# Somedaywilldo/BM-NAS

Hardware: AMD Instinct MI355X
Metric: search-steps/sec (fwd+bwd of fusion hypernet) on MM-IMDB synthetic (higher is better)
Workload: dtype f32; 1 GPU; mmimdb fusion search, batch 128 per GPU x 1 GPU(s), N6 C192 L16 steps2 node_steps1 node_multiplier1, train mode, dropout 0.1/0.1(attn); inputs=(b, C, L) features, global_batch=128, per_gpu_batch=128, parallelism=dp1, mode=graph, step=fwd+bwd, one hipGraph replay

## Files before the change

bm-nas_amd/csrc/common.hpp:

```cpp
#pragma once
#include <hip/hip_runtime.h>
#include <stdint.h>

#define BMNAS_MAX_PTRS 16
#define BMNAS_WAVE 64

typedef __attribute__((ext_vector_type(4))) float f32x4;

struct PtrsIn { const float* p[BMNAS_MAX_PTRS]; };
struct PtrsOut { float* p[BMNAS_MAX_PTRS]; };

struct DropCfg {
  uint32_t thr;
  float scale;
  uint64_t seed;
  uint64_t offset;
  const uint64_t* step;
};

#define BMNAS_CHECK_LAUNCH()                         \
  do {                                               \
    hipError_t e__ = hipGetLastError();              \
    if (e__ != hipSuccess) return (int)e__;          \
  } while (0)

__device__ __forceinline__ uint4 philox4x32_10(uint64_t ctr, uint64_t seed) {
  uint32_t k0 = (uint32_t)seed, k1 = (uint32_t)(seed >> 32);
  uint32_t c0 = (uint32_t)ctr, c1 = (uint32_t)(ctr >> 32), c2 = 0x2545F491u, c3 = 0x9E3779B1u;
#pragma unroll
  for (int r = 0; r < 10; ++r) {
    uint32_t hi0 = __umulhi(0xD2511F53u, c0), lo0 = 0xD2511F53u * c0;
    uint32_t hi1 = __umulhi(0xCD9E8D57u, c2), lo1 = 0xCD9E8D57u * c2;
    uint32_t n0 = hi1 ^ c1 ^ k0, n1 = lo1, n2 = hi0 ^ c3 ^ k1, n3 = lo0;
    c0 = n0; c1 = n1; c2 = n2; c3 = n3;
    k0 += 0x9E3779B9u; k1 += 0xBB67AE85u;
  }
  return make_uint4(c0, c1, c2, c3);
}

struct DropRt {
  uint32_t thr;
  float scale;
  uint64_t seed;
  uint64_t off;
};
__device__ __forceinline__ DropRt drop_begin(const DropCfg& d) {
  DropRt r{d.thr, d.scale, d.seed, d.offset};
  if (d.thr != 0u && d.step != nullptr) r.off += d.step[0];
  return r;
}
__device__ __forceinline__ float4 drop_mult4(const DropRt& d, uint64_t e) {
  if (d.thr == 0u) return make_float4(1.f, 1.f, 1.f, 1.f);
  uint4 r = philox4x32_10(d.off + (e >> 2), d.seed);
  return make_float4(r.x >= d.thr ? d.scale : 0.f, r.y >= d.thr ? d.scale : 0.f,
                     r.z >= d.thr ? d.scale : 0.f, r.w >= d.thr ? d.scale : 0.f);
}

__device__ __forceinline__ float4 drop_mult4(const DropCfg& d, uint64_t e) {
  if (d.thr == 0u) return make_float4(1.f, 1.f, 1.f, 1.f);
  const uint64_t base = (d.step != nullptr) ? d.step[0] : 0ull;
  uint4 r = philox4x32_10(base + d.offset + (e >> 2), d.seed);
  return make_float4(r.x >= d.thr ? d.scale : 0.f, r.y >= d.thr ? d.scale : 0.f,
                     r.z >= d.thr ? d.scale : 0.f, r.w >= d.thr ? d.scale : 0.f);
}

#ifndef BMNAS_BODY_PROBES
#define BMNAS_BODY_PROBES 0
#endif
#if BMNAS_BODY_PROBES
static __device__ unsigned long long* g_bmnas_stamps = nullptr;
static __device__ int g_bmnas_stamp_slots = 0;
#define BMNAS_DEFINE_STAMP_SETTER(name)                                                                   \
  extern "C" int name(void* buf, int slots) {                                                             \
    unsigned long long* p = reinterpret_cast<unsigned long long*>(buf);                                   \
    if (hipMemcpyToSymbol(HIP_SYMBOL(g_bmnas_stamps), &p, sizeof(p)) != hipSuccess) return -1;            \
    if (hipMemcpyToSymbol(HIP_SYMBOL(g_bmnas_stamp_slots), &slots, sizeof(slots)) != hipSuccess) return -1; \
    return 0;                                                                                             \
  }
__device__ __forceinline__ unsigned long long stamp_clock() {
  unsigned long long t;
  asm volatile("s_memtime %0\n\ts_waitcnt lgkmcnt(0)" : "=s"(t)::"memory");
  return t;
}
__device__ __forceinline__ unsigned long long stamp_wall() {
  unsigned long long t;
  asm volatile("s_memrealtime %0\n\ts_waitcnt lgkmcnt(0)" : "=s"(t)::"memory");
  return t;
}
#define STAMP(slot, wg, i)                                                                         \
  do {                                                                                             \
    __builtin_amdgcn_sched_barrier(0);                                                             \
    if (threadIdx.x == 0 && g_bmnas_stamps != nullptr && (wg) < g_bmnas_stamp_slots) {             \
      unsigned long long* p__ = g_bmnas_stamps + ((size_t)(slot) * g_bmnas_stamp_slots + (wg)) * 8; \
      p__[i] = stamp_clock();                                                                      \
      if ((i) == 0) p__[6] = stamp_wall();                                                         \
      p__[7] = stamp_wall();                                                                       \
    }                                                                                              \
    __builtin_amdgcn_sched_barrier(0);                                                             \
  } while (0)
#else
#define STAMP(slot, wg, i) do { } while (0)
#define BMNAS_DEFINE_STAMP_SETTER(name) \
  extern "C" int name(void* buf, int slots) { (void)buf; (void)slots; return -3;  }
#endif

template <int CTRL>
__device__ __forceinline__ float dpp_f(float v) {
  return __int_as_float(__builtin_amdgcn_update_dpp(__float_as_int(v), __float_as_int(v), CTRL, 0xf, 0xf, false));
}
__device__ __forceinline__ float lane_xor1(float v) { return dpp_f<0xB1>(v); }
__device__ __forceinline__ float lane_xor2(float v) { return dpp_f<0x4E>(v); }
__device__ __forceinline__ float xor16_sum(float v) {
  auto r = __builtin_amdgcn_permlane16_swap(__float_as_uint(v), __float_as_uint(v), false, false);
  return __uint_as_float(r[0]) + __uint_as_float(r[1]);
}
__device__ __forceinline__ float xor32_sum(float v) {
  auto r = __builtin_amdgcn_permlane32_swap(__float_as_uint(v), __float_as_uint(v), false, false);
  return __uint_as_float(r[0]) + __uint_as_float(r[1]);
}
__device__ __forceinline__ float xor16_max(float v) {
  auto r = __builtin_amdgcn_permlane16_swap(__float_as_uint(v), __float_as_uint(v), false, false);
  return fmaxf(__uint_as_float(r[0]), __uint_as_float(r[1]));
}
__device__ __forceinline__ float xor32_max(float v) {
  auto r = __builtin_amdgcn_permlane32_swap(__float_as_uint(v), __float_as_uint(v), false, false);
  return fmaxf(__uint_as_float(r[0]), __uint_as_float(r[1]));
}
__device__ __forceinline__ float row_stride4_sum(float v) {
  v += dpp_f<0x124>(v);
  v += dpp_f<0x128>(v);
  return v;
}
__device__ __forceinline__ float row16_sum(float v) {
// ... 35 lines not shown

template <int NW>
__device__ __forceinline__ float block_sum_fresh(float v, float* red) {
  v = wave_sum(v);
  if ((threadIdx.x & 63) == 0) red[threadIdx.x >> 6] = v;
  __syncthreads();
  float t = red[0];
#pragma unroll
  for (int i = 1; i < NW; ++i) t += red[i];
  return t;
}

template <int NW, int N>
__device__ __forceinline__ void block_sum_lead_fresh(float (&v)[N], float* red) {
#pragma unroll
  for (int i = 0; i < N; ++i) v[i] = wave_sum(v[i]);
  const int w = threadIdx.x >> 6;
  if ((threadIdx.x & 63) == 0) {
#pragma unroll
    for (int i = 0; i < N; ++i) red[i * NW + w] = v[i];
  }
  __syncthreads();
  float t = red[0];
#pragma unroll
  for (int k = 1; k < NW; ++k) t += red[k];
  v[0] = t;
  if (threadIdx.x == 0) {
#pragma unroll
    for (int i = 1; i < N; ++i) {
      float u = red[i * NW];
#pragma unroll
      for (int k = 1; k < NW; ++k) u += red[i * NW + k];
      v[i] = u;
    }
  }
}

template <int NW, int N>
__device__ __forceinline__ void block_sum_n(float (&v)[N], float* red) {
#pragma unroll
  for (int i = 0; i < N; ++i) v[i] = wave_sum(v[i]);
  const int w = threadIdx.x >> 6;
  __syncthreads();
  if ((threadIdx.x & 63) == 0) {
#pragma unroll
    for (int i = 0; i < N; ++i) red[w * N + i] = v[i];
  }
  __syncthreads();
#pragma unroll
  for (int i = 0; i < N; ++i) {
    float t = red[i];
#pragma unroll
    for (int k = 1; k < NW; ++k) t += red[k * N + i];
    v[i] = t;
  }
}

template <int NW, int N>
__device__ __forceinline__ void block_sum_lead(float (&v)[N], float* red) {
  __syncthreads();
  block_sum_lead_fresh<NW, N>(v, red);
}

template <typename T>
__device__ __forceinline__ T* sgpr_ptr(T* p) {
  asm volatile("" : "+s"(p));
  return p;
}
template <typename T, int N>
__device__ __forceinline__ T* pick_ptr(T* const (&arr)[N], int q) {
  T* p = sgpr_ptr(arr[0]);
#pragma unroll
  for (int qq = 1; qq < N; ++qq) {
    T* c = sgpr_ptr(arr[qq]);
    p = (q == qq) ? c : p;
  }
  return p;
}

__device__ __forceinline__ float4 ld4(const float* p) { return *reinterpret_cast<const float4*>(p); }
__device__ __forceinline__ void st4(float* p, float4 v) { *reinterpret_cast<float4*>(p) = v; }
__device__ __forceinline__ void pin4(float4& v) { asm volatile("" : "+v"(v.x), "+v"(v.y), "+v"(v.z), "+v"(v.w)); }
__device__ __forceinline__ void pin1(float& v) { asm volatile("" : "+v"(v)); }

__device__ __forceinline__ void st4_wt(float* p, float4 v) {
#if defined(BMNAS_NO_WT)
  *reinterpret_cast<float4*>(p) = v;
#else
  const f32x4 d = {v.x, v.y, v.z, v.w};
  asm volatile("global_store_dwordx4 %0, %1, off sc1\n\ts_nop 1" : : "v"(p), "v"(d) : "memory");
#endif
}

#ifndef BMNAS_WT_MASK
#define BMNAS_WT_MASK 0x29
#endif
template <int G>
__device__ __forceinline__ void st4_wtg(float* p, float4 v) {
  if constexpr ((BMNAS_WT_MASK >> G) & 1) st4_wt(p, v);
  else *reinterpret_cast<float4*>(p) = v;
}

#ifndef BMNAS_WT0_MASK
#define BMNAS_WT0_MASK 0x7FF
#endif
template <int K>
__device__ __forceinline__ void st4_w0(float* p, float4 v) {
  if constexpr ((BMNAS_WT0_MASK >> K) & 1) st4_wt(p, v);
  else *reinterpret_cast<float4*>(p) = v;
}

__device__ __forceinline__ void st16_wt(void* p, uint4 v) {
#if defined(BMNAS_NO_WT) || !((BMNAS_WT_MASK >> 5) & 1)
  *reinterpret_cast<uint4*>(p) = v;
#else
  typedef __attribute__((ext_vector_type(4))) unsigned u32x4_;
  const u32x4_ d = {v.x, v.y, v.z, v.w};
  asm volatile("global_store_dwordx4 %0, %1, off sc1\n\ts_nop 1" : : "v"(p), "v"(d) : "memory");
#endif
}

__device__ __forceinline__ float4 f4_add(float4 a, float4 b) {
  return make_float4(a.x + b.x, a.y + b.y, a.z + b.z, a.w + b.w);
}
__device__ __forceinline__ float4 f4_mul(float4 a, float4 b) {
  return make_float4(a.x * b.x, a.y * b.y, a.z * b.z, a.w * b.w);
}
__device__ __forceinline__ float4 f4_scale(float4 a, float s) {
  return make_float4(a.x * s, a.y * s, a.z * s, a.w * s);
}
__device__ __forceinline__ float f4_dot(float4 a, float4 b) {
  return a.x * b.x + a.y * b.y + a.z * b.z + a.w * b.w;
}
__device__ __forceinline__ float f4_hsum(float4 a) { return (a.x + a.y) + (a.z + a.w); }

static inline int ilog2_exact(int v) {
  int l = 0;
  while ((1 << l) < v) ++l;
  return ((1 << l) == v) ? l : -1;
}
```

bm-nas_amd/csrc/head.hip:

```cpp
#include "common.hpp"
#include "../../include/bmnas_hip.h"
#include "lazy_ln.hpp"
#include "ln_sample.hpp"
#include <algorithm>
#include <cstdlib>

namespace {

constexpr int kHeadSrc = 4;
constexpr int kMaxO = 128;

struct HeadSrc {
  const float* p[kHeadSrc];
  const float* sums[kHeadSrc];
};

struct HeadLazy {
  const float* rec;
  const float* prm;
  const float* nw[kHeadSrc];
  const float* nb[kHeadSrc];
  float* nstats[kHeadSrc];
  float* lnpart[kHeadSrc];
  int lq, P;
};

__device__ __forceinline__ void sample_stats(const HeadSrc& src, int n_src, int s, int D, float* mean, float* rstd) {
  float S = 0.f, Q = 0.f;
  float2 sv[kHeadSrc];
#pragma unroll
  for (int q = 0; q < kHeadSrc; ++q)
    sv[q] = reinterpret_cast<const float2*>(pick_ptr(src.sums, q < n_src ? q : 0))[s];
#pragma unroll
  for (int q = 0; q < kHeadSrc; ++q) {
    S += q < n_src ? sv[q].x : 0.f;
    Q += q < n_src ? sv[q].y : 0.f;
  }
  const float inv = 1.f / (float)D;
  const float m = S * inv;
  const float var = fmaxf(Q * inv - m * m, 0.f);
  *mean = m;
  *rstd = 1.f / sqrtf(var + kLnEps);
}

struct HeadFwdArgs {
  HeadSrc src;
  const float* ln_w;
  const float* ln_b;
  const float* W;
  const float* bias;
  float* hb;
  float* hb_part;
  long long hb_stride;
  float* stats;
  int b, O, D, CL, n_src, KS;
};

template <int J, int TJ, bool LZ>
__global__ __launch_bounds__(256) void head_fwd_k(HeadFwdArgs a, HeadLazy z) {
  __shared__ float red[4][3][16][16 * TJ + 1];
  const int wave = threadIdx.x >> 6, lane = threadIdx.x & 63;
  const int lo = lane & 15, h = lane >> 4;
  const int ks = blockIdx.x, st = blockIdx.y;
  STAMP(4, blockIdx.y * gridDim.x + blockIdx.x, 0);
  const int s = st * 16 + lo;
  const int sc = s < a.b ? s : a.b - 1;
  const int nkb = a.D / 16;
  int oc[TJ];
#pragma unroll
  for (int t = 0; t < TJ; ++t) {
    const int o = 16 * t + lo;
    oc[t] = o < a.O ? o : a.O - 1;
  }
  float4 xv[J], lw[J], lb[J], wv[J][TJ], nwv[LZ ? J : 1], nbv[LZ ? J : 1];
  bool valid[J], lzq[J];
#pragma unroll
  for (int j = 0; j < J; ++j) {
    const int kb = (j * a.KS + ks) * 4 + wave;
    valid[j] = kb < nkb;
    const int kbc = valid[j] ? kb : nkb - 1;
    const int k = kbc * 16 + 4 * h;
    const int q = (kbc * 16) / a.CL;
    xv[j] = ld4(pick_ptr(a.src.p, q) + (int64_t)sc * a.CL + (k - q * a.CL));
    lw[j] = ld4(a.ln_w + k);
    lb[j] = ld4(a.ln_b + k);
    lzq[j] = LZ && q == z.lq;
    if (LZ) {
      nwv[j] = ld4(lzq[j] ? z.nw[0] + (k - q * a.CL) : a.ln_w + k);
      nbv[j] = ld4(lzq[j] ? z.nb[0] + (k - q * a.CL) : a.ln_b + k);
    }
#pragma unroll
    for (int t = 0; t < TJ; ++t) wv[j][t] = ld4(a.W + (int64_t)oc[t] * a.D + k);
  }
  __builtin_amdgcn_sched_barrier(0);
  float mean, rstd, nmean = 0.f, nrstd = 1.f;
  if (LZ) {
    float2 sv[kHeadSrc];
#pragma unroll
    for (int q = 0; q < kHeadSrc; ++q) {
      const bool use = q < a.n_src && q != z.lq;
      const int qq = use ? q : (z.lq == 0 ? (a.n_src > 1 ? 1 : 0) : 0);
      const float* sp = pick_ptr(a.src.sums, qq);
      sv[q] = reinterpret_cast<const float2*>(sp != nullptr ? sp : z.rec)[sc];
    }
    const LazyStats ls = lazy_combine(z.rec, z.prm, z.P, sc);
    float S = ls.osum, Q = ls.osq;
#pragma unroll
    for (int q = 0; q < kHeadSrc; ++q) {
      const bool use = q < a.n_src && q != z.lq;
      S += use ? sv[q].x : 0.f;
      Q += use ? sv[q].y : 0.f;
    }
    const float inv = 1.f / (float)a.D;
    mean = S * inv;
    rstd = 1.f / sqrtf(fmaxf(Q * inv - mean * mean, 0.f) + kLnEps);
    nmean = ls.mean;
    nrstd = ls.rstd;
  } else {
    sample_stats(a.src, a.n_src, sc, a.D, &mean, &rstd);
  }
  if (ks == 0 && wave == 0 && h == 0 && s < a.b) {
    a.stats[2 * s] = mean;
    a.stats[2 * s + 1] = rstd;
    if (LZ) {
      z.nstats[0][2 * s] = nmean;
      z.nstats[0][2 * s + 1] = nrstd;
    }
  }
  STAMP(4, blockIdx.y * gridDim.x + blockIdx.x, 1);
  __builtin_amdgcn_sched_barrier(0);
  f32x4 acc[3][TJ];
#pragma unroll
  for (int v = 0; v < 3; ++v)
#pragma unroll
    for (int t = 0; t < TJ; ++t) acc[v][t] = (f32x4){0.f, 0.f, 0.f, 0.f};
#pragma unroll
  for (int j = 0; j < J; ++j) {
    if (!valid[j]) continue;
    float x4[4] = {xv[j].x, xv[j].y, xv[j].z, xv[j].w};
    const float w4[4] = {lw[j].x, lw[j].y, lw[j].z, lw[j].w};
    const float b4[4] = {lb[j].x, lb[j].y, lb[j].z, lb[j].w};
    if (LZ && lzq[j]) {
      const float n4[4] = {nwv[j].x, nwv[j].y, nwv[j].z, nwv[j].w};
      const float c4[4] = {nbv[j].x, nbv[j].y, nbv[j].z, nbv[j].w};
#pragma unroll
      for (int r = 0; r < 4; ++r) x4[r] = ln_apply(x4[r], nmean, nrstd, n4[r], c4[r]);
    }
#pragma unroll
    for (int r = 0; r < 4; ++r) {
      const float xh = ln_xhat(x4[r], mean, rstd);
      const float pre = xh * w4[r] + b4[r];
      const bool on = pre > 0.f;
      const float f = on ? pre : 0.f;
      const float a2 = on ? w4[r] : 0.f;
      const float a3 = a2 * xh;
#pragma unroll
      for (int t = 0; t < TJ; ++t) {
        const float wr = r == 0 ? wv[j][t].x : r == 1 ? wv[j][t].y : r == 2 ? wv[j][t].z : wv[j][t].w;
        acc[0][t] = __builtin_amdgcn_mfma_f32_16x16x4f32(f, wr, acc[0][t], 0, 0, 0);
        acc[1][t] = __builtin_amdgcn_mfma_f32_16x16x4f32(a2, wr, acc[1][t], 0, 0, 0);
        acc[2][t] = __builtin_amdgcn_mfma_f32_16x16x4f32(a3, wr, acc[2][t], 0, 0, 0);
      }
    }
  }
#pragma unroll
  for (int v = 0; v < 3; ++v)
#pragma unroll
    for (int t = 0; t < TJ; ++t)
#pragma unroll
      for (int r = 0; r < 4; ++r) red[wave][v][4 * h + r][16 * t + lo] = acc[v][t][r];
  STAMP(4, blockIdx.y * gridDim.x + blockIdx.x, 2);
  __syncthreads();
  const int rows = (a.b - st * 16) < 16 ? (a.b - st * 16) : 16;
  const int per_v = rows * a.O;
  for (int i = threadIdx.x; i < 3 * per_v; i += 256) {
    const int v = i / per_v, e = i - v * per_v;
    const int sr = e / a.O, o = e - sr * a.O;
    float val = (red[0][v][sr][o] + red[1][v][sr][o]) + (red[2][v][sr][o] + red[3][v][sr][o]);
    if (v == 0 && ks == 0) val += a.bias[o];
    if (a.hb_part != nullptr) a.hb_part[(int64_t)ks * a.hb_stride + ((int64_t)v * a.b + st * 16) * a.O + e] = val;
    else atomicAdd(a.hb + ((int64_t)v * a.b + st * 16) * a.O + e, val);
  }
  STAMP(4, blockIdx.y * gridDim.x + blockIdx.x, 3);
}

struct HeadBwdArgs {
  HeadSrc src;
  float* dsrc[kHeadSrc];
  uint32_t acc_mask;
  const float* ln_w;
  const float* ln_b;
  const float* W;
  const float* hb;
  const float* stats;
  const float* g;
  const float* gscale;
  const float* labels_f;
  const long long* labels_i;
  float* loss;
  float* loss_part;
  float* part;
  float* scrub;
  long long scrub4;
  int b, O, D, CL, n_src, mode;
  int probe;
  const float* cw;
  const float* cpw;
  long long ignore;
  float eps;
  int red;
};

__device__ __forceinline__ float sigmoidf_(float v) { return 1.f / (1.f + __expf(-v)); }

__device__ __forceinline__ float group16_sum(float v) { return row16_sum(v); }
__device__ __forceinline__ float group16_max(float v) { return row16_max(v); }

template <int OT, int SG, bool LZ, int CR = 0>
__global__ __launch_bounds__(256) void head_bwd_k(HeadBwdArgs a, HeadLazy z) {
  constexpr int kSteps = 4 * OT, kRows = 16 * SG;
  constexpr int kDlA = 4 * kSteps + 4, kMs = LZ ? 8 : 4;
  __shared__ __attribute__((aligned(16))) float dl_a[kRows][kDlA];
  __shared__ __attribute__((aligned(16))) float dl_b[kRows / 4][16 * OT][4];
  __shared__ __attribute__((aligned(16))) float ms[kRows][kMs];
  __shared__ __attribute__((aligned(16))) float ft_s[4][SG][16][20];
  __shared__ float lnp_s[LZ ? 4 : 1][LZ ? kRows : 1][2];
  __shared__ float loss_s[4];
  const int wave = threadIdx.x >> 6, lane = threadIdx.x & 63;
  const int lo = lane & 15, h = lane >> 4;
  const int chunk = blockIdx.y, s0 = chunk * kRows;
  STAMP(5, blockIdx.y * gridDim.x + blockIdx.x, 0);
  const float gs = (a.gscale != nullptr) ? a.gscale[0] : 1.f;
  const float invD = 1.f / (float)a.D;
  const int nkt = a.D / 16;
  const int kt = blockIdx.x * 4 + wave;
  const bool vt = kt < nkt;
  const int k0 = (vt ? kt : nkt - 1) * 16;
  const int q = k0 / a.CL;
  const int kin = k0 - q * a.CL;
  float wv[kSteps];
#pragma unroll
  for (int t = 0; t < kSteps; ++t) {
    const int o = 4 * t + h;
    wv[t] = a.W[(int64_t)(o < a.O ? o : a.O - 1) * a.D + k0 + lo];
  }
  const float4 lw = ld4(a.ln_w + k0 + 4 * h), lb = ld4(a.ln_b + k0 + 4 * h);
  const float* const srcq = pick_ptr(a.src.p, q);
  float4 nw4 = make_float4(1.f, 1.f, 1.f, 1.f), nb4 = make_float4(0.f, 0.f, 0.f, 0.f);
  const float* nstq = nullptr;
  if (LZ) {
    const float* const nwq_p = pick_ptr(z.nw, q);
    const float* const nbq_p = pick_ptr(z.nb, q);
    nstq = pick_ptr(z.nstats, q);
    nw4 = ld4(nwq_p + kin + 4 * h);
    nb4 = ld4(nbq_p + kin + 4 * h);
  }
  float4 x[SG];
#pragma unroll
  for (int g = 0; g < SG; ++g) {
    const int s = s0 + 16 * g + lo;
    x[g] = ld4(srcq + (int64_t)(s < a.b ? s : a.b - 1) * a.CL + kin + 4 * h);
  }
  {
    float zz[SG][OT], aa[SG][OT], bb[SG][OT], yy[SG][OT], st_mean[SG], st_rstd[SG], nd_mean[SG], nd_rstd[SG];
// ... 626 lines not shown
```

bm-nas_amd/csrc/lazy_ln.hpp:

```cpp
#pragma once
#include "common.hpp"
#include "ln_sample.hpp"

constexpr int kLazyPart = 256;
constexpr int kLazyMaxParts = 4;
constexpr int kLazyRec = 8;

struct LazyStats {
  float mean, rstd, osum, osq;
};

__host__ __device__ inline int lazy_parts(int cl4) { return (cl4 + kLazyPart - 1) / kLazyPart; }

__device__ __forceinline__ LazyStats lazy_combine(const float* __restrict__ rec, const float* __restrict__ prm,
                                                  const int P, const int s) {
  float4 ra[kLazyMaxParts], rb[kLazyMaxParts], pa[kLazyMaxParts], pb[kLazyMaxParts];
#pragma unroll
  for (int k = 0; k < kLazyMaxParts; ++k) {
    const int kc = k < P ? k : 0;
    const float* r = rec + ((int64_t)s * P + kc) * kLazyRec;
    ra[k] = ld4(r);
    rb[k] = ld4(r + 4);
    pa[k] = ld4(prm + kc * kLazyRec);
    pb[k] = ld4(prm + kc * kLazyRec + 4);
  }
  float D = 0.f, sm = 0.f;
#pragma unroll
  for (int k = 0; k < kLazyMaxParts; ++k) {
    const float n = k < P ? pb[k].y : 0.f;
    D += n;
    sm += n * ra[k].x;
  }
  const float mu = sm / D;
  float M2 = 0.f, S1 = 0.f, S2 = 0.f, S3 = 0.f, H = 0.f, I = 0.f;
#pragma unroll
  for (int k = 0; k < kLazyMaxParts; ++k) {
    if (k < P) {
      const float d = ra[k].x - mu;
      M2 += ra[k].y + pb[k].y * d * d;
      S1 += ra[k].z + d * pa[k].y;
      S2 += ra[k].w + 2.f * d * rb[k].y + d * d * pa[k].x;
      S3 += rb[k].x + d * pa[k].z;
      H += pa[k].w;
      I += pb[k].x;
    }
  }
  LazyStats o;
  o.mean = mu;
  o.rstd = 1.f / sqrtf(M2 / D + kLnEps);
  o.osum = o.rstd * S1 + H;
  o.osq = o.rstd * o.rstd * S2 + 2.f * o.rstd * S3 + I;
  return o;
}
```

bm-nas_amd/csrc/lazyln.hip:

```cpp
#include "common.hpp"
#include "../../include/bmnas_hip.h"
#include "bn_fin.hpp"
#include "lazy_ln.hpp"
#include "mix_common.hpp"

namespace {

__global__ __launch_bounds__(256) void node_mix_pre_fwd_k(
    const float* __restrict__ x, const float* __restrict__ y, const float* __restrict__ p1,
    const float* __restrict__ U, float* __restrict__ chan, BnFin fin, const float* __restrict__ gamma,
    const float* __restrict__ resid, const float* __restrict__ ln_w, const float* __restrict__ ln_b,
    float* __restrict__ pre, float* __restrict__ rec, float* __restrict__ prm, int b, int C, int L,
    DropCfg dglu, DropCfg dfc) {
  __shared__ float red[4];
  __shared__ float red5[2 * 4 * 5];
  extern __shared__ float fin_lds[];
  const int cl4 = C * L / 4, l4n = L / 4, M = 3 * C;
  const int part = blockIdx.x, smp = blockIdx.y, P = gridDim.x;
  STAMP(0, smp * P + part, 0);
  float* sc = fin_lds;
  float* sh = fin_lds + M;
  const int r0 = part * kLazyPart + threadIdx.x;
  const bool act = r0 < cl4;
  const int r = act ? r0 : cl4 - 1;
// ... 5 lines not shown
  const float4 xv = ld4(x + e), yv = ld4(y + e), pv = ld4(p1 + e), rv = ld4(resid + e);
  __builtin_amdgcn_sched_barrier(0);
  const float g0 = gamma[0], g1 = gamma[1], g2 = gamma[2], g3 = gamma[3];
  const DropRt rglu = drop_begin(dglu), rfc = drop_begin(dfc);
  STAMP(0, smp * P + part, 1);
  bn_fin_fill<256>(fin, chan, M, b * L, sc, sh, part == 0 && smp == 0);
  STAMP(0, smp * P + part, 2);
  const float4 va = affine4(ua, sc[c], sh[c]);
  const float4 vg = affine4(ug, sc[C + c], sh[C + c]);
  const float4 vf = affine4(uf, sc[2 * C + c], sh[2 * C + c]);
  const float4 m2 = drop_mult4(rglu, (uint64_t)e), m3 = drop_mult4(rfc, (uint64_t)e);
  const float4 o = mix_fwd4<kMixAll>(g0, g1, g2, g3, f4_add(xv, yv), pv, va, vg, vf, m2, m3);
  const float4 v = f4_add(o, rv);
  if (act) st4_w0<3>(pre + e, v);
  STAMP(0, smp * P + part, 3);
  const int n4 = cl4 - part * kLazyPart < kLazyPart ? cl4 - part * kLazyPart : kLazyPart;
  const float nk = (float)(4 * n4);
  float mk = wave_sum(act ? f4_hsum(v) : 0.f);
  const int wv = threadIdx.x >> 6, ln = threadIdx.x & 63;
  if (ln == 0) red[wv] = mk;
  __syncthreads();
  mk = (((red[0] + red[1]) + red[2]) + red[3]) / nk;
  float acc[5] = {0.f, 0.f, 0.f, 0.f, 0.f};
  if (act) {
    const float4 cd = make_float4(v.x - mk, v.y - mk, v.z - mk, v.w - mk);
    const float4 cw = f4_mul(cd, lw);
    acc[0] = f4_dot(cd, cd);
    acc[1] = f4_hsum(cw);
    acc[2] = f4_dot(cw, cw);
    acc[3] = f4_dot(cw, lb);
    acc[4] = f4_dot(cw, lw);
  }
  float pa[5] = {0.f, 0.f, 0.f, 0.f, 0.f};
  if (smp == 0 && act) {
    pa[0] = f4_dot(lw, lw);
    pa[1] = f4_hsum(lw);
    pa[2] = f4_dot(lw, lb);
    pa[3] = f4_hsum(lb);
    pa[4] = f4_dot(lb, lb);
  }
#pragma unroll
  for (int i = 0; i < 5; ++i) acc[i] = wave_sum(acc[i]);
  if (smp == 0) {
#pragma unroll
    for (int i = 0; i < 5; ++i) pa[i] = wave_sum(pa[i]);
  }
  if (ln == 0) {
#pragma unroll
    for (int i = 0; i < 5; ++i) red5[i * 4 + wv] = acc[i];
    if (smp == 0) {
#pragma unroll
      for (int i = 0; i < 5; ++i) red5[20 + i * 4 + wv] = pa[i];
    }
  }
  __syncthreads();
  if (threadIdx.x == 0) {
    float t[5];
#pragma unroll
    for (int i = 0; i < 5; ++i) t[i] = ((red5[i * 4] + red5[i * 4 + 1]) + red5[i * 4 + 2]) + red5[i * 4 + 3];
    float* rr = rec + ((int64_t)smp * P + part) * kLazyRec;
    st4(rr, make_float4(mk, t[0], t[1], t[2]));
    st4(rr + 4, make_float4(t[3], t[4], 0.f, 0.f));
  }
  STAMP(0, smp * P + part, 4);
  if (smp == 0 && threadIdx.x == 64) {
    float t[5];
#pragma unroll
    for (int i = 0; i < 5; ++i)
      t[i] = ((red5[20 + i * 4] + red5[20 + i * 4 + 1]) + red5[20 + i * 4 + 2]) + red5[20 + i * 4 + 3];
    st4(prm + part * kLazyRec, make_float4(t[0], t[1], t[2], t[3]));
    st4(prm + part * kLazyRec + 4, make_float4(t[4], nk, 0.f, 0.f));
  }
}

template <int NIN>
__global__ __launch_bounds__(256) void mixsum_pair_fwd_lazy_k(
    PtrsIn xs, const float* __restrict__ w, int w_stride, const float* __restrict__ w2, int w2_stride,
    const float* __restrict__ pre, const float* __restrict__ rec, const float* __restrict__ prm,
    const float* __restrict__ ln_w, const float* __restrict__ ln_b, float* __restrict__ nout,
    float* __restrict__ stats, float* __restrict__ osum, float* __restrict__ out, float* __restrict__ out2,
    int cl4) {
  const int part = blockIdx.x, smp = blockIdx.y, P = gridDim.x;
  STAMP(1, smp * P + part, 0);
  const int r0 = part * kLazyPart + threadIdx.x;
  const bool act = r0 < cl4;
  const int r = act ? r0 : cl4 - 1;
  const int64_t i = (int64_t)smp * cl4 + r;
  float wj[NIN + 1];
#pragma unroll
  for (int j = 0; j <= NIN; ++j) wj[j] = w[j * w_stride];
  const float s2 = w2[0] + w2[w2_stride];
  float4 v[NIN];
#pragma unroll
  for (int j = 0; j < NIN; ++j) v[j] = reinterpret_cast<const float4*>(xs.p[j])[i];
  const float4 pv = reinterpret_cast<const float4*>(pre)[i];
  const float4 lw = ld4(ln_w + (int64_t)r * 4), lb = ld4(ln_b + (int64_t)r * 4);
  const LazyStats st = lazy_combine(rec, prm, P, smp);
  const float4 n = ln_apply4(pv, st.mean, st.rstd, lw, lb);
  float4 acc = f4_scale(v[0], wj[0]);
#pragma unroll
  for (int j = 1; j < NIN; ++j) {
    acc.x = fmaf(wj[j], v[j].x, acc.x);
    acc.y = fmaf(wj[j], v[j].y, acc.y);
    acc.z = fmaf(wj[j], v[j].z, acc.z);
    acc.w = fmaf(wj[j], v[j].w, acc.w);
  }
  acc.x = fmaf(wj[NIN], n.x, acc.x);
  acc.y = fmaf(wj[NIN], n.y, acc.y);
  acc.z = fmaf(wj[NIN], n.z, acc.z);
  acc.w = fmaf(wj[NIN], n.w, acc.w);
  if (act) {
    st4_w0<4>(nout + 4 * i, n);
    st4_w0<4>(out + 4 * i, acc);
    st4_w0<4>(out2 + 4 * i, f4_scale(acc, s2));
  }
  STAMP(1, smp * P + part, 1);
  if (part == 0 && threadIdx.x == 0) {
    stats[2 * smp] = st.mean;
    stats[2 * smp + 1] = st.rstd;
    if (osum != nullptr) {
      osum[2 * smp] = st.osum;
      osum[2 * smp + 1] = st.osq;
    }
  }
}

constexpr int kMaxLazyIn = 2;
struct LazyIn {
  const float* pre[kMaxLazyIn];
  const float* ln_w[kMaxLazyIn];
  const float* stats[kMaxLazyIn];
  float* lnpart[kMaxLazyIn];
  int stride[kMaxLazyIn];
};

template <int NIN, int NLZ, bool DOTS = true>
__global__ __launch_bounds__(256) void mixsum_pair_bwd_lazy_k(
    PtrsIn xs, PtrsOut dxs, const float* __restrict__ w, int w_stride, const float* __restrict__ w2, int w2_stride,
    const float* __restrict__ h, const float* __restrict__ gh, const float* __restrict__ gz,
    const float* __restrict__ gz2, float* dw, float* dw2, int dw_shards, int64_t dw_shard_stride, uint32_t acc_mask,
    LazyIn Z, float* __restrict__ g_full, int cl4) {
  constexpr int NR = NIN + 1 + 2 * NLZ;
  __shared__ float red[4 * NR];
  const int part = blockIdx.x, smp = blockIdx.y, P = gridDim.x;
  STAMP(2, smp * P + part, 0);
  const int r0 = part * kLazyPart + threadIdx.x;
  const bool act = r0 < cl4;
  const int r = act ? r0 : cl4 - 1;
  const int64_t i = (int64_t)smp * cl4 + r;
  float wj[NIN];
#pragma unroll
  for (int j = 0; j < NIN; ++j) wj[j] = w[j * w_stride];
  const float s2 = w2[0] + w2[w2_stride];
  const float4 zero4 = make_float4(0.f, 0.f, 0.f, 0.f);
  float4 z4 = reinterpret_cast<const float4*>(gz)[i];
  const float4 z2v = reinterpret_cast<const float4*>(gz2 != nullptr ? gz2 : gz)[i];
  float4 h4 = zero4;
  if constexpr (DOTS) h4 = reinterpret_cast<const float4*>(h)[i];
  const float4 ghv = reinterpret_cast<const float4*>(gh != nullptr ? gh : gz)[i];
  float4 v[NIN];
#pragma unroll
  for (int j = 0; j < NIN; ++j) {
    if constexpr (DOTS) v[j] = reinterpret_cast<const float4*>(xs.p[j])[i];
    else v[j] = zero4;
  }
  z4 = f4_add(z4, gz2 != nullptr ? z2v : zero4);
  float4 g4 = f4_add(f4_scale(z4, s2), gh != nullptr ? ghv : zero4);
  float4 pz[NLZ], lz[NLZ], oldn[NLZ];
  float mean[NLZ], rstd[NLZ];
#pragma unroll
  for (int t = 0; t < NLZ; ++t) {
    pz[t] = reinterpret_cast<const float4*>(Z.pre[t])[i];
    lz[t] = ld4(Z.ln_w[t] + (int64_t)r * 4);
    mean[t] = Z.stats[t][2 * smp];
    rstd[t] = Z.stats[t][2 * smp + 1];
    const float* od = dxs.p[NIN - NLZ + t];
    oldn[t] = reinterpret_cast<const float4*>(od != nullptr && (acc_mask & (1u << (NIN - NLZ + t))) ? od : gz)[i];
  }
  if (!act) {
    z4 = make_float4(0.f, 0.f, 0.f, 0.f);
// ... 386 lines not shown
```

Baseline: 7370 steps/s.

## Load lazy-LN records via scalar loads and hoist head bias reads

Splits lazy_combine into issue, pin and finish stages. In the mixsum kernel the per-sample records and mixing weights go through the constant address space (scalar loads) and are pinned in SGPRs, with kernel arguments marked scalar. The head kernel issues its record loads early and pins them in VGPRs, and it prefetches bias values before the reduction barrier, splitting the output loop so only the first component adds bias. Contraction control keeps the arithmetic identical between the uniform and per-lane variants, at the cost of more inline-asm register constraints that may raise register pressure.

After: 7414 steps/s (median of 4 runs). No clear change (+0.6%).

```diff
diff --git a/bm-nas_amd/csrc/common.hpp b/bm-nas_amd/csrc/common.hpp
--- a/bm-nas_amd/csrc/common.hpp
+++ b/bm-nas_amd/csrc/common.hpp
@@ -1,6 +1,7 @@
 #pragma once
 #include <hip/hip_runtime.h>
 #include <stdint.h>
+#include <type_traits>
 
 #define BMNAS_MAX_PTRS 16
 #define BMNAS_WAVE 64
@@ -49,6 +50,11 @@
   if (d.thr != 0u && d.step != nullptr) r.off += d.step[0];
   return r;
 }
+__device__ __forceinline__ float mul_nc(const float a, const float b) {
+#pragma clang fp contract(off)
+  return a * b;
+}
+
 __device__ __forceinline__ float4 drop_mult4(const DropRt& d, uint64_t e) {
   if (d.thr == 0u) return make_float4(1.f, 1.f, 1.f, 1.f);
   uint4 r = philox4x32_10(d.off + (e >> 2), d.seed);
@@ -250,6 +256,29 @@
 __device__ __forceinline__ void st4(float* p, float4 v) { *reinterpret_cast<float4*>(p) = v; }
 __device__ __forceinline__ void pin4(float4& v) { asm volatile("" : "+v"(v.x), "+v"(v.y), "+v"(v.z), "+v"(v.w)); }
 __device__ __forceinline__ void pin1(float& v) { asm volatile("" : "+v"(v)); }
+template <typename T>
+__device__ __forceinline__ void spin(T& v) {
+  static_assert((sizeof(T) == 4 || sizeof(T) == 8) && !std::is_pointer<T>::value, "one or two SGPRs of data");
+  asm volatile("" : "+s"(v));
+}
+template <typename T>
+__device__ __forceinline__ void sarg(const T& v) {
+  static_assert(sizeof(T) == 4 || sizeof(T) == 8, "one or two SGPRs");
+  asm volatile("" : : "s"(v));
+}
+template <typename T>
+__device__ __forceinline__ T ldk(const T* p) {
+  return *reinterpret_cast<const __attribute__((address_space(4))) T*>(reinterpret_cast<uintptr_t>(p));
+}
+__device__ __forceinline__ float4 ldk4(const float* p) {
+  const f32x4 t = ldk(reinterpret_cast<const f32x4*>(p));
+  return make_float4(t[0], t[1], t[2], t[3]);
+}
+__device__ __forceinline__ float2 ldk2(const float* p) {
+  typedef __attribute__((ext_vector_type(2))) float v2;
+  const v2 t = ldk(reinterpret_cast<const v2*>(p));
+  return make_float2(t[0], t[1]);
+}
 
 __device__ __forceinline__ void st4_wt(float* p, float4 v) {
 #if defined(BMNAS_NO_WT)
diff --git a/bm-nas_amd/csrc/head.hip b/bm-nas_amd/csrc/head.hip
--- a/bm-nas_amd/csrc/head.hip
+++ b/bm-nas_amd/csrc/head.hip
@@ -103,7 +103,9 @@
       const float* sp = pick_ptr(a.src.sums, qq);
       sv[q] = reinterpret_cast<const float2*>(sp != nullptr ? sp : z.rec)[sc];
     }
-    const LazyStats ls = lazy_combine(z.rec, z.prm, z.P, sc);
+    LazyRecs lrq = lazy_issue(z.rec, z.prm, z.P, sc);
+    lazy_pin(lrq);
+    const LazyStats ls = lazy_finish<true>(lrq, z.P);
     float S = ls.osum, Q = ls.osq;
 #pragma unroll
     for (int q = 0; q < kHeadSrc; ++q) {
@@ -163,6 +165,14 @@
       }
     }
   }
+  const int rows = (a.b - st * 16) < 16 ? (a.b - st * 16) : 16;
+  const int per_v = rows * a.O;
+  float bq[TJ];
+#pragma unroll
+  for (int t = 0; t < TJ; ++t) {
+    const int i = (int)threadIdx.x + 256 * t;
+    bq[t] = a.bias[(i < per_v ? i : per_v - 1) % a.O];
+  }
 #pragma unroll
   for (int v = 0; v < 3; ++v)
 #pragma unroll
@@ -171,15 +181,21 @@
       for (int r = 0; r < 4; ++r) red[wave][v][4 * h + r][16 * t + lo] = acc[v][t][r];
   STAMP(4, blockIdx.y * gridDim.x + blockIdx.x, 2);
   __syncthreads();
-  const int rows = (a.b - st * 16) < 16 ? (a.b - st * 16) : 16;
-  const int per_v = rows * a.O;
-  for (int i = threadIdx.x; i < 3 * per_v; i += 256) {
-    const int v = i / per_v, e = i - v * per_v;
+  auto tile_out = [&](const int v, const int e, const bool biased, const float bv) {
     const int sr = e / a.O, o = e - sr * a.O;
     float val = (red[0][v][sr][o] + red[1][v][sr][o]) + (red[2][v][sr][o] + red[3][v][sr][o]);
-    if (v == 0 && ks == 0) val += a.bias[o];
+    if (biased) val += bv;
     if (a.hb_part != nullptr) a.hb_part[(int64_t)ks * a.hb_stride + ((int64_t)v * a.b + st * 16) * a.O + e] = val;
     else atomicAdd(a.hb + ((int64_t)v * a.b + st * 16) * a.O + e, val);
+  };
+#pragma unroll
+  for (int t = 0; t < TJ; ++t) {
+    const int i = (int)threadIdx.x + 256 * t;
+    if (i < per_v) tile_out(0, i, ks == 0, bq[t]);
+  }
+  for (int i = per_v + threadIdx.x; i < 3 * per_v; i += 256) {
+    const int v = i / per_v;
+    tile_out(v, i - v * per_v, false, 0.f);
   }
   STAMP(4, blockIdx.y * gridDim.x + blockIdx.x, 3);
 }
diff --git a/bm-nas_amd/csrc/lazy_ln.hpp b/bm-nas_amd/csrc/lazy_ln.hpp
--- a/bm-nas_amd/csrc/lazy_ln.hpp
+++ b/bm-nas_amd/csrc/lazy_ln.hpp
@@ -12,18 +12,105 @@
 
 __host__ __device__ inline int lazy_parts(int cl4) { return (cl4 + kLazyPart - 1) / kLazyPart; }
 
-__device__ __forceinline__ LazyStats lazy_combine(const float* __restrict__ rec, const float* __restrict__ prm,
-                                                  const int P, const int s) {
-  float4 ra[kLazyMaxParts], rb[kLazyMaxParts], pa[kLazyMaxParts], pb[kLazyMaxParts];
+struct LazyRecs {
+  float4 ra[kLazyMaxParts], pa[kLazyMaxParts];
+  float2 rb[kLazyMaxParts], pb[kLazyMaxParts];
+};
+
+template <bool UNIFORM = false>
+__device__ __forceinline__ LazyRecs lazy_issue(const float* __restrict__ rec, const float* __restrict__ prm,
+                                               const int P, const int s) {
+  LazyRecs q;
 #pragma unroll
   for (int k = 0; k < kLazyMaxParts; ++k) {
     const int kc = k < P ? k : 0;
     const float* r = rec + ((int64_t)s * P + kc) * kLazyRec;
-    ra[k] = ld4(r);
-    rb[k] = ld4(r + 4);
-    pa[k] = ld4(prm + kc * kLazyRec);
-    pb[k] = ld4(prm + kc * kLazyRec + 4);
+    const float* m = prm + kc * kLazyRec;
+    if constexpr (UNIFORM) {
+      q.ra[k] = ldk4(r);
+      q.rb[k] = ldk2(r + 4);
+      q.pa[k] = ldk4(m);
+      q.pb[k] = ldk2(m + 4);
+    } else {
+      q.ra[k] = ld4(r);
+      q.rb[k] = *reinterpret_cast<const float2*>(r + 4);
+      q.pa[k] = ld4(m);
+      q.pb[k] = *reinterpret_cast<const float2*>(m + 4);
+    }
   }
+  return q;
+}
+
+typedef __attribute__((ext_vector_type(2))) float f32x2;
+#define BMNAS_LAZY_PIN_OPS(c_)                                                                                       \
+  c_(a[0]), c_(a[1]), c_(a[2]), c_(a[3]), c_(a[4]), c_(a[5]), c_(a[6]), c_(a[7]), c_(c[0]), c_(c[1]), c_(c[2]), c_(c[3]), \
+      c_(c[4]), c_(c[5]), c_(c[6]), c_(c[7])
+#define BMNAS_LAZY_S(x_) "+s"(x_)
+#define BMNAS_LAZY_V(x_) "+v"(x_)
+static_assert(kLazyMaxParts == 4, "BMNAS_LAZY_PIN_OPS lists sixteen operands");
+struct LazyPinRegs {
+  f32x4 a[2 * kLazyMaxParts];
+  f32x2 c[2 * kLazyMaxParts];
+  __device__ __forceinline__ explicit LazyPinRegs(const LazyRecs& q) {
+#pragma unroll
+    for (int k = 0; k < kLazyMaxParts; ++k) {
+      a[2 * k] = (f32x4){q.ra[k].x, q.ra[k].y, q.ra[k].z, q.ra[k].w};
+      a[2 * k + 1] = (f32x4){q.pa[k].x, q.pa[k].y, q.pa[k].z, q.pa[k].w};
+      c[2 * k] = (f32x2){q.rb[k].x, q.rb[k].y};
+      c[2 * k + 1] = (f32x2){q.pb[k].x, q.pb[k].y};
+    }
+  }
+  __device__ __forceinline__ void out(LazyRecs& q) const {
+#pragma unroll
+    for (int k = 0; k < kLazyMaxParts; ++k) {
+      q.ra[k] = make_float4(a[2 * k][0], a[2 * k][1], a[2 * k][2], a[2 * k][3]);
+      q.pa[k] = make_float4(a[2 * k + 1][0], a[2 * k + 1][1], a[2 * k + 1][2], a[2 * k + 1][3]);
+      q.rb[k] = make_float2(c[2 * k][0], c[2 * k][1]);
+      q.pb[k] = make_float2(c[2 * k + 1][0], c[2 * k + 1][1]);
+    }
+  }
+};
+
+__device__ __forceinline__ void lazy_pin(LazyRecs& q) {
+  LazyPinRegs r(q);
+  f32x4(&a)[2 * kLazyMaxParts] = r.a;
+  f32x2(&c)[2 * kLazyMaxParts] = r.c;
+  asm volatile("" : BMNAS_LAZY_PIN_OPS(BMNAS_LAZY_V));
+  r.out(q);
+}
+
+template <int N>
+__device__ __forceinline__ void lazy_pin_with(LazyRecs& q, float (&w)[N]) {
+  static_assert(N >= 1 && N <= 20, "up to 20 floats beside the records");
+  LazyPinRegs r(q);
+  f32x4(&a)[2 * kLazyMaxParts] = r.a;
+  f32x2(&c)[2 * kLazyMaxParts] = r.c;
+  constexpr int W = N <= 4 ? 4 : N <= 8 ? 8 : 16;
+  typedef float __attribute__((ext_vector_type(W))) wide_t;
+  wide_t t;
+  f32x4 u;
+#pragma unroll
+  for (int i = 0; i < W; ++i) t[i] = w[i < N ? i : 0];
+#pragma unroll
+  for (int i = 0; i < 4; ++i) u[i] = w[16 + i < N ? 16 + i : 0];
+  if constexpr (N <= 16) asm volatile("" : "+s"(t), BMNAS_LAZY_PIN_OPS(BMNAS_LAZY_S));
+  else asm volatile("" : "+s"(t), "+s"(u), BMNAS_LAZY_PIN_OPS(BMNAS_LAZY_S));
+#pragma unroll
+  for (int i = 0; i < W; ++i)
+    if (i < N) w[i] = t[i];
+#pragma unroll
+  for (int i = 0; i < 4; ++i)
+    if (16 + i < N) w[16 + i] = u[i];
+  r.out(q);
+}
+#undef BMNAS_LAZY_PIN_OPS
+#undef BMNAS_LAZY_S
+#undef BMNAS_LAZY_V
+
+template <bool PER_LANE>
+__device__ __forceinline__ LazyStats lazy_finish(const LazyRecs& q, const int P) {
+  const float4 (&ra)[kLazyMaxParts] = q.ra, (&pa)[kLazyMaxParts] = q.pa;
+  const float2 (&rb)[kLazyMaxParts] = q.rb, (&pb)[kLazyMaxParts] = q.pb;
   float D = 0.f, sm = 0.f;
 #pragma unroll
   for (int k = 0; k < kLazyMaxParts; ++k) {
@@ -35,20 +122,28 @@
   float M2 = 0.f, S1 = 0.f, S2 = 0.f, S3 = 0.f, H = 0.f, I = 0.f;
 #pragma unroll
   for (int k = 0; k < kLazyMaxParts; ++k) {
-    if (k < P) {
-      const float d = ra[k].x - mu;
-      M2 += ra[k].y + pb[k].y * d * d;
-      S1 += ra[k].z + d * pa[k].y;
-      S2 += ra[k].w + 2.f * d * rb[k].y + d * d * pa[k].x;
-      S3 += rb[k].x + d * pa[k].z;
-      H += pa[k].w;
-      I += pb[k].x;
-    }
+    const bool on = k < P;
+    const float d = ra[k].x - mu;
+    const float t_m2 = ra[k].y + pb[k].y * d * d;
+    const float t_s1 = ra[k].z + d * pa[k].y;
+    const float t_s2 = ra[k].w + 2.f * d * rb[k].y + d * d * pa[k].x;
+    const float t_s3 = rb[k].x + d * pa[k].z;
+    M2 += on ? t_m2 : 0.f;
+    S1 += on ? t_s1 : 0.f;
+    S2 += on ? t_s2 : 0.f;
+    S3 += on ? t_s3 : 0.f;
+    H += on ? pa[k].w : 0.f;
+    I += on ? pb[k].x : 0.f;
   }
   LazyStats o;
   o.mean = mu;
   o.rstd = 1.f / sqrtf(M2 / D + kLnEps);
-  o.osum = o.rstd * S1 + H;
-  o.osq = o.rstd * o.rstd * S2 + 2.f * o.rstd * S3 + I;
+  if constexpr (PER_LANE) {
+    o.osum = __builtin_fmaf(o.rstd, S1, H);
+    o.osq = __builtin_fmaf(o.rstd * o.rstd, S2, mul_nc(2.f * o.rstd, S3)) + I;
+  } else {
+    o.osum = mul_nc(o.rstd, S1) + H;
+    o.osq = __builtin_fmaf(2.f * o.rstd, S3, mul_nc(o.rstd * o.rstd, S2)) + I;
+  }
   return o;
 }
diff --git a/bm-nas_amd/csrc/lazyln.hip b/bm-nas_amd/csrc/lazyln.hip
--- a/bm-nas_amd/csrc/lazyln.hip
+++ b/bm-nas_amd/csrc/lazyln.hip
@@ -111,20 +111,29 @@
     int cl4) {
   const int part = blockIdx.x, smp = blockIdx.y, P = gridDim.x;
   STAMP(1, smp * P + part, 0);
+#pragma unroll
+  for (int j = 0; j < NIN; ++j) sarg(xs.p[j]);
+  sarg(w); sarg(w_stride); sarg(w2); sarg(w2_stride); sarg(pre); sarg(rec); sarg(prm); sarg(ln_w); sarg(ln_b);
+  sarg(nout); sarg(stats); sarg(osum); sarg(out); sarg(out2); sarg(cl4);
   const int r0 = part * kLazyPart + threadIdx.x;
   const bool act = r0 < cl4;
   const int r = act ? r0 : cl4 - 1;
   const int64_t i = (int64_t)smp * cl4 + r;
-  float wj[NIN + 1];
-#pragma unroll
-  for (int j = 0; j <= NIN; ++j) wj[j] = w[j * w_stride];
-  const float s2 = w2[0] + w2[w2_stride];
   float4 v[NIN];
 #pragma unroll
   for (int j = 0; j < NIN; ++j) v[j] = reinterpret_cast<const float4*>(xs.p[j])[i];
   const float4 pv = reinterpret_cast<const float4*>(pre)[i];
   const float4 lw = ld4(ln_w + (int64_t)r * 4), lb = ld4(ln_b + (int64_t)r * 4);
-  const LazyStats st = lazy_combine(rec, prm, P, smp);
+  __builtin_amdgcn_sched_barrier(0);
+  float wj[NIN + 3];
+#pragma unroll
+  for (int j = 0; j <= NIN; ++j) wj[j] = ldk(w + j * w_stride);
+  wj[NIN + 1] = ldk(w2);
+  wj[NIN + 2] = ldk(w2 + w2_stride);
+  LazyRecs lrq = lazy_issue<true>(rec, prm, P, smp);
+  lazy_pin_with(lrq, wj);
+  const float s2 = wj[NIN + 1] + wj[NIN + 2];
+  const LazyStats st = lazy_finish<false>(lrq, P);
   const float4 n = ln_apply4(pv, st.mean, st.rstd, lw, lb);
   float4 acc = f4_scale(v[0], wj[0]);
 #pragma unroll
```

## Compute head LN stats once per block and share affine params via LDS

Applied to the files above, without the earlier changes.

The head forward kernel now has only the last 16 threads compute per-sample LayerNorm statistics, and a subset of threads load the LN affine weights. Both are shared through LDS, so the redundant per-lane statistics work and affine global loads go away. It also replaces the division used to find the source index with comparisons, folds the bias into the accumulator init, stores the reduction tile compactly so the final pass is unrolled with division-free indexing, and defers the stats writes to the end. This adds an extra __syncthreads and some LDS traffic, and it relies on a static thread-range assumption.

After: 7351 steps/s before, 7370 steps/s after (median of 3 runs). No clear change (+0.3%).

```diff
diff --git a/bm-nas_amd/csrc/head.hip b/bm-nas_amd/csrc/head.hip
--- a/bm-nas_amd/csrc/head.hip
+++ b/bm-nas_amd/csrc/head.hip
@@ -58,82 +58,134 @@
 
 template <int J, int TJ, bool LZ>
 __global__ __launch_bounds__(256) void head_fwd_k(HeadFwdArgs a, HeadLazy z) {
-  __shared__ float red[4][3][16][16 * TJ + 1];
-  const int wave = threadIdx.x >> 6, lane = threadIdx.x & 63;
+  constexpr int kNV = LZ ? 4 : 2;
+  constexpr int kAff = 16 * J;
+  constexpr int kStat0 = 240;
+  constexpr int kTile = 3 * 16 * 16 * TJ;
+  constexpr int kTrips = kTile / 256;
+  static_assert(kNV * kAff <= kStat0, "affine and statistics threads overlap");
+  __shared__ float red[4][kTile];
+  __shared__ __attribute__((aligned(16))) float4 aff_s[kNV * kAff];
+  __shared__ __attribute__((aligned(16))) float4 stat_s[16];
+  const int tid = threadIdx.x;
+  const int wave = __builtin_amdgcn_readfirstlane(tid >> 6), lane = tid & 63;
   const int lo = lane & 15, h = lane >> 4;
   const int ks = blockIdx.x, st = blockIdx.y;
   STAMP(4, blockIdx.y * gridDim.x + blockIdx.x, 0);
   const int s = st * 16 + lo;
   const int sc = s < a.b ? s : a.b - 1;
-  const int nkb = a.D / 16;
+  const int nkb = (int)((unsigned)a.D >> 4);
+  const int cl2 = a.n_src > 2 ? 2 * a.CL : a.D, cl3 = a.n_src > 3 ? 3 * a.CL : a.D;
   int oc[TJ];
 #pragma unroll
   for (int t = 0; t < TJ; ++t) {
     const int o = 16 * t + lo;
     oc[t] = o < a.O ? o : a.O - 1;
   }
-  float4 xv[J], lw[J], lb[J], wv[J][TJ], nwv[LZ ? J : 1], nbv[LZ ? J : 1];
+  float4 xv[J], wv[J][TJ];
+  float bv[TJ];
   bool valid[J], lzq[J];
 #pragma unroll
   for (int j = 0; j < J; ++j) {
     const int kb = (j * a.KS + ks) * 4 + wave;
     valid[j] = kb < nkb;
-    const int kbc = valid[j] ? kb : nkb - 1;
-    const int k = kbc * 16 + 4 * h;
-    const int q = (kbc * 16) / a.CL;
-    xv[j] = ld4(pick_ptr(a.src.p, q) + (int64_t)sc * a.CL + (k - q * a.CL));
-    lw[j] = ld4(a.ln_w + k);
-    lb[j] = ld4(a.ln_b + k);
+    const int k0 = (valid[j] ? kb : nkb - 1) * 16;
+    const int q = (k0 >= a.CL) + (k0 >= cl2) + (k0 >= cl3);
+    xv[j] = ld4(pick_ptr(a.src.p, q) + (int64_t)sc * a.CL + (k0 - q * a.CL + 4 * h));
     lzq[j] = LZ && q == z.lq;
+#pragma unroll
+    for (int t = 0; t < TJ; ++t) wv[j][t] = ld4(a.W + (int64_t)oc[t] * a.D + k0 + 4 * h);
+  }
+#pragma unroll
+  for (int t = 0; t < TJ; ++t) bv[t] = a.bias[oc[t]];
+  float4 affv;
+  {
+    const int i = tid < kNV * kAff ? tid : 0;
+    const int vec = i / kAff, r = i - vec * kAff;
+    const int w = r / (4 * J), j = (r >> 2) - w * J, hh = r & 3;
+    const int kb = (j * a.KS + ks) * 4 + w;
+    const int k0 = (kb < nkb ? kb : nkb - 1) * 16, k = k0 + 4 * hh;
+    const float* const w7 = sgpr_ptr(a.ln_w);
+    const float* const b7 = sgpr_ptr(a.ln_b);
+    const float* base = (vec & 1) ? b7 : w7;
+    int off = k;
     if (LZ) {
-      nwv[j] = ld4(lzq[j] ? z.nw[0] + (k - q * a.CL) : a.ln_w + k);
-      nbv[j] = ld4(lzq[j] ? z.nb[0] + (k - q * a.CL) : a.ln_b + k);
-    }
-#pragma unroll
-    for (int t = 0; t < TJ; ++t) wv[j][t] = ld4(a.W + (int64_t)oc[t] * a.D + k);
+      const float* const wn = sgpr_ptr(z.nw[0]);
+      const float* const bn = sgpr_ptr(z.nb[0]);
+      const int q = (k0 >= a.CL) + (k0 >= cl2) + (k0 >= cl3);
+      const bool node = vec >= 2 && q == z.lq;
+      const float* const nbase = (vec & 1) ? bn : wn;
+      base = node ? nbase : base;
+      off = node ? k - q * a.CL : k;
+    }
+    affv = ld4(base + off);
   }
   __builtin_amdgcn_sched_barrier(0);
-  float mean, rstd, nmean = 0.f, nrstd = 1.f;
-  if (LZ) {
-    float2 sv[kHeadSrc];
-#pragma unroll
-    for (int q = 0; q < kHeadSrc; ++q) {
-      const bool use = q < a.n_src && q != z.lq;
-      const int qq = use ? q : (z.lq == 0 ? (a.n_src > 1 ? 1 : 0) : 0);
-      const float* sp = pick_ptr(a.src.sums, qq);
-      sv[q] = reinterpret_cast<const float2*>(sp != nullptr ? sp : z.rec)[sc];
-    }
-    const LazyStats ls = lazy_combine(z.rec, z.prm, z.P, sc);
-    float S = ls.osum, Q = ls.osq;
-#pragma unroll
-    for (int q = 0; q < kHeadSrc; ++q) {
-      const bool use = q < a.n_src && q != z.lq;
-      S += use ? sv[q].x : 0.f;
-      Q += use ? sv[q].y : 0.f;
-    }
-    const float inv = 1.f / (float)a.D;
-    mean = S * inv;
-    rstd = 1.f / sqrtf(fmaxf(Q * inv - mean * mean, 0.f) + kLnEps);
-    nmean = ls.mean;
-    nrstd = ls.rstd;
-  } else {
-    sample_stats(a.src, a.n_src, sc, a.D, &mean, &rstd);
-  }
-  if (ks == 0 && wave == 0 && h == 0 && s < a.b) {
-    a.stats[2 * s] = mean;
-    a.stats[2 * s + 1] = rstd;
+  float mean = 0.f, rstd = 0.f, nmean = 0.f, nrstd = 1.f;
+  if (tid >= kStat0) {
     if (LZ) {
-      z.nstats[0][2 * s] = nmean;
-      z.nstats[0][2 * s + 1] = nrstd;
-    }
-  }
+      float2 sv[kHeadSrc];
+#pragma unroll
+      for (int q = 0; q < kHeadSrc; ++q) {
+        const bool use = q < a.n_src && q != z.lq;
+        const int qq = use ? q : (z.lq == 0 ? (a.n_src > 1 ? 1 : 0) : 0);
+        const float* sp = pick_ptr(a.src.sums, qq);
+        sv[q] = reinterpret_cast<const float2*>(sp != nullptr ? sp : z.rec)[sc];
+      }
+      const LazyStats ls = lazy_combine(z.rec, z.prm, z.P, sc);
+      float S = ls.osum, Q = ls.osq;
+#pragma unroll
+      for (int q = 0; q < kHeadSrc; ++q) {
+        const bool use = q < a.n_src && q != z.lq;
+        S += use ? sv[q].x : 0.f;
+        Q += use ? sv[q].y : 0.f;
+      }
+      const float inv = 1.f / (float)a.D;
+      mean = S * inv;
+      rstd = 1.f / sqrtf(fmaxf(Q * inv - mean * mean, 0.f) + kLnEps);
+      nmean = ls.mean;
+      nrstd = ls.rstd;
+    } else {
+      sample_stats(a.src, a.n_src, sc, a.D, &mean, &rstd);
+    }
+    stat_s[tid - kStat0] = make_float4(mean, rstd, nmean, nrstd);
+  }
+  if (tid < kNV * kAff) aff_s[tid] = affv;
+  __syncthreads();
+  float4 sv4 = stat_s[lo];
+  float4 lw[J], lb[J], nwv[LZ ? J : 1], nbv[LZ ? J : 1];
+#pragma unroll
+  for (int j = 0; j < J; ++j) {
+    const int i = (wave * J + j) * 4 + h;
+    lw[j] = aff_s[i];
+    lb[j] = aff_s[kAff + i];
+    if (LZ) {
+      nwv[j] = aff_s[2 * kAff + i];
+      nbv[j] = aff_s[3 * kAff + i];
+    }
+  }
+  pin4(sv4);
+#pragma unroll
+  for (int j = 0; j < J; ++j) {
+    pin4(lw[j]);
+    pin4(lb[j]);
+    if (LZ) {
+      pin4(nwv[j]);
+      pin4(nbv[j]);
+    }
+  }
+  mean = sv4.x; rstd = sv4.y; nmean = sv4.z; nrstd = sv4.w;
   STAMP(4, blockIdx.y * gridDim.x + blockIdx.x, 1);
   __builtin_amdgcn_sched_barrier(0);
+  const bool bias_here = ks == 0 && wave == 0;
   f32x4 acc[3][TJ];
 #pragma unroll
-  for (int v = 0; v < 3; ++v)
-#pragma unroll
-    for (int t = 0; t < TJ; ++t) acc[v][t] = (f32x4){0.f, 0.f, 0.f, 0.f};
+  for (int t = 0; t < TJ; ++t) {
+    const float b0 = bias_here ? bv[t] : 0.f;
+    acc[0][t] = (f32x4){b0, b0, b0, b0};
+    acc[1][t] = (f32x4){0.f, 0.f, 0.f, 0.f};
+    acc[2][t] = (f32x4){0.f, 0.f, 0.f, 0.f};
+  }
 #pragma unroll
   for (int j = 0; j < J; ++j) {
     if (!valid[j]) continue;
@@ -163,23 +215,61 @@
       }
     }
   }
-#pragma unroll
-  for (int v = 0; v < 3; ++v)
-#pragma unroll
-    for (int t = 0; t < TJ; ++t)
-#pragma unroll
-      for (int r = 0; r < 4; ++r) red[wave][v][4 * h + r][16 * t + lo] = acc[v][t][r];
+  const int rows = (a.b - st * 16) < 16 ? (a.b - st * 16) : 16;
+  const int per_v = rows * a.O, tot = 3 * per_v;
+  {
+    float* const my = red[wave];
+#pragma unroll
+    for (int t = 0; t < TJ; ++t) {
+      const int o = 16 * t + lo;
+      if (o < a.O) {
+#pragma unroll
+        for (int r = 0; r < 4; ++r) {
+          const int sr = 4 * h + r;
+          if (sr < rows) {
+#pragma unroll
+            for (int v = 0; v < 3; ++v) my[v * per_v + sr * a.O + o] = acc[v][t][r];
+          }
+        }
+      }
+    }
+  }
   STAMP(4, blockIdx.y * gridDim.x + blockIdx.x, 2);
   __syncthreads();
-  const int rows = (a.b - st * 16) < 16 ? (a.b - st * 16) : 16;
-  const int per_v = rows * a.O;
-  for (int i = threadIdx.x; i < 3 * per_v; i += 256) {
-    const int v = i / per_v, e = i - v * per_v;
-    const int sr = e / a.O, o = e - sr * a.O;
-    float val = (red[0][v][sr][o] + red[1][v][sr][o]) + (red[2][v][sr][o] + red[3][v][sr][o]);
-    if (v == 0 && ks == 0) val += a.bias[o];
-    if (a.hb_part != nullptr) a.hb_part[(int64_t)ks * a.hb_stride + ((int64_t)v * a.b + st * 16) * a.O + e] = val;
-    else atomicAdd(a.hb + ((int64_t)v * a.b + st * 16) * a.O + e, val);
+  float pv[kTrips][4];
+#pragma unroll
+  for (int n = 0; n < kTrips; ++n) {
+    const int i = tid + 256 * n;
+    const int ic = i < tot ? i : 0;
+#pragma unroll
+    for (int w = 0; w < 4; ++w) pv[n][w] = red[w][ic];
+  }
+#pragma unroll
+  for (int n = 0; n < kTrips; ++n)
+#pragma unroll
+    for (int w = 0; w < 4; ++w) pin1(pv[n][w]);
+  float* const dst = (a.hb_part != nullptr ? a.hb_part + (int64_t)ks * a.hb_stride : a.hb) + (int64_t)st * 16 * a.O;
+  const int64_t dv = (int64_t)a.b * a.O - per_v;
+  const bool part = a.hb_part != nullptr;
+  auto trips = [&](auto put) {
+#pragma unroll
+    for (int n = 0; n < kTrips; ++n) {
+      const int i = tid + 256 * n;
+      if (i < tot) {
+        const int v = (i >= per_v) + (i >= 2 * per_v);
+        put(dst + (i + v * dv), (pv[n][0] + pv[n][1]) + (pv[n][2] + pv[n][3]));
+      }
+    }
+  };
+  if (part) trips([](float* p, float val) { *p = val; });
+  else trips([](float* p, float val) { atomicAdd(p, val); });
+  if (tid >= kStat0 && ks == 0 && s < a.b) {
+    a.stats[2 * s] = mean;
+    a.stats[2 * s + 1] = rstd;
+    if (LZ) {
+      z.nstats[0][2 * s] = nmean;
+      z.nstats[0][2 * s + 1] = nrstd;
+    }
   }
   STAMP(4, blockIdx.y * gridDim.x + blockIdx.x, 3);
 }
```
